# chenbinghui1/DSL

Hardware: AMD Instinct MI355X
Metric: imgs/sec training step, FCOS R50-FPN 1333x800 (higher is better)
Workload: dtype bf16; 1 GPU; FCOS R50-caffe-FPN supervised training step (BASELINE.json configs[1]), 2 x (3,800,1344) per GPU, synthetic COCO-shaped boxes, random-init weights; global_batch=2, parallelism=dp1, optimizer=SGD momentum 0.9 wd 1e-4

## Files before the change

### dsl_amd/build.py

```python
import os
import subprocess
import sys
from concurrent.futures import ThreadPoolExecutor

HERE = os.path.dirname(os.path.abspath(__file__))
CSRC = os.path.join(HERE, 'csrc')
LIBDIR = os.path.join(HERE, 'lib')
LIB = os.path.join(LIBDIR, 'libdsl_hip.so')
SOURCES = ['api.hip', 'conv.hip', 'wgrad.hip', 'misc.hip', 'fcos_loss.hip', 'optim.hip', 'detect.hip', 'rla.hip', 'datapath.hip', 'comm.hip', 'stem.hip', 'bneck.hip']
FLAGS = ['--offload-arch=gfx950', '-O3', '-std=c++17', '-fPIC', '-Wno-unused-result', '-Wno-unused-value']


def _hipcc():
    for c in (os.environ.get('HIPCC'), '/opt/rocm/bin/hipcc', 'hipcc'):
        if c and (os.path.isabs(c) and os.path.exists(c) or not os.path.isabs(c)):
            return c
    raise RuntimeError('hipcc not found')


def _stale(out, deps):
    if not os.path.exists(out):
        return True
    t = os.path.getmtime(out)
    return any(os.path.getmtime(d) > t for d in deps)


def build_lib(force=False, verbose=True):
    os.makedirs(LIBDIR, exist_ok=True)
    hdrs = [os.path.join(CSRC, 'common.hpp'), os.path.join(HERE, '..', 'include', 'dsl_hip.h')]
    srcs = [os.path.join(CSRC, s) for s in SOURCES if os.path.exists(os.path.join(CSRC, s))]
    objs = [os.path.join(LIBDIR, os.path.basename(s)[:-4] + '.o') for s in srcs]
    hipcc = _hipcc()

    def compile_one(so):
        s, o = so
        if force or _stale(o, [s] + hdrs):
            cmd = [hipcc] + FLAGS + ['-c', s, '-o', o]
            if verbose:
                print(' '.join(cmd), flush=True)
            subprocess.check_call(cmd)
        return o

    with ThreadPoolExecutor(max_workers=6) as ex:
        list(ex.map(compile_one, zip(srcs, objs)))
    if force or _stale(LIB, objs):
        cmd = [hipcc, '--offload-arch=gfx950', '-shared', '-fPIC', '-Wl,--no-undefined'] + objs + ['-ldl', '-o', LIB]
        if verbose:
            print(' '.join(cmd), flush=True)
        subprocess.check_call(cmd)
    return LIB


if __name__ == '__main__':
    build_lib(force='--force' in sys.argv)
    print(LIB)
```

### dsl_amd/csrc/conv.hip

```cpp
#include <stdlib.h>
#include <algorithm>

#include <mutex>
#include <type_traits>
#include <vector>

#include "common.hpp"

namespace {

constexpr int BPX = 128;
constexpr int BK = 64;

struct ConvK {
  int nseg, n;
  int gh[DSL_MAX_SEG], gw[DSL_MAX_SEG], sh[DSL_MAX_SEG], sw[DSL_MAX_SEG];
  int dh[DSL_MAX_SEG], dw[DSL_MAX_SEG], ah[DSL_MAX_SEG], aw[DSL_MAX_SEG];
  int pxstart[DSL_MAX_SEG + 1];
  long long soff[DSL_MAX_SEG], doff[DSL_MAX_SEG], aoff[DSL_MAX_SEG];
  int cs, cd, ldd, lda, ldm, kh, kw, stride, pad, mode, os, flags;
  int lds;
  int ktiles, kc;
  int ident;
  int addfast;
  int dbg;
  int splits, kt_per_split, cd_pad;
  int gx, gy, xcd_chunk;
  float* ws;
  long long wrow;
  const uint16_t* src;
  const uint16_t* wgt;
  void* dst;
  const float* scale;
  const float* bias;
  const uint16_t* addend;
  const uint16_t* mask;
  float* gnws;
  const uint16_t* gnx;
  const float* gngamma;
  const float* gnbeta;
  const float* gnstats;
};

__device__ __forceinline__ u32x4 relu_bf16x8(u32x4 v) {
#pragma unroll
  for (int i = 0; i < 4; ++i) {
    uint32_t w = v[i];
    uint32_t neg = (w >> 15) & 0x00010001u;
    v[i] = w & ~(neg * 0xffffu);
  }
  return v;
}

struct PixRow {
  long long base;
  int y, x, sh, sw;
  bool ok;
};

__device__ __forceinline__ void lds_barrier() {
  asm volatile("s_waitcnt lgkmcnt(0)\n\ts_barrier" ::: "memory");
}

__device__ __forceinline__ void decode_pixel(const ConvK& p, int gp, int& seg, int& img, int& y, int& x) {
  seg = 0;
#pragma unroll
  for (int s = 1; s < DSL_MAX_SEG; ++s)
    if (s < p.nseg && gp >= p.pxstart[s]) seg = s;
  const int q = gp - p.pxstart[seg];
  const int hw = p.gh[seg] * p.gw[seg];
  img = q / hw;
  const int rem = q - img * hw;
  y = rem / p.gw[seg];
  x = rem - y * p.gw[seg];
}


__device__ __forceinline__ void conv_epilogue4(const ConvK& p, long long dpix, long long apix, int co, float v[4]) {
  const bool out_f32 = (p.flags & DSL_CONV_OUT_F32) != 0;
  const bool relu_out = (p.flags & DSL_CONV_RELU_OUT) != 0;
  const bool mask_first = (p.flags & DSL_CONV_MASK_FIRST) != 0 && p.mask != nullptr;
  const bool mask_last = (p.flags & DSL_CONV_MASK_LAST) != 0 && p.mask != nullptr;
  const bool has_mask = mask_first || mask_last;
  if (co + 3 < p.cd) {
    if (p.scale) {
      const f32x4 s4 = *reinterpret_cast<const f32x4*>(p.scale + co);
#pragma unroll
      for (int e = 0; e < 4; ++e) v[e] *= s4[e];
    }
    if (p.bias) {
      const f32x4 b4 = *reinterpret_cast<const f32x4*>(p.bias + co);
#pragma unroll
      for (int e = 0; e < 4; ++e) v[e] += b4[e];
    }
    float m[4] = {1.f, 1.f, 1.f, 1.f};
    if (has_mask) {
      const u32x2 mm = *reinterpret_cast<const u32x2*>(p.mask + dpix * p.ldm + co);
      m[0] = bflo(mm[0]) > 0.f ? 1.f : 0.f;
      m[1] = bfhi(mm[0]) > 0.f ? 1.f : 0.f;
// ... 199 lines not shown
    for (int i = 0; i < 8; ++i) v[i] = fmaxf(v[i], 0.f);
  }
  const u32x4 o = {pack2bf(v[0], v[1]), pack2bf(v[2], v[3]), pack2bf(v[4], v[5]), pack2bf(v[6], v[7])};
  *reinterpret_cast<u32x4*>(e.dst + (long long)gp * e.ldd) = o;
}

__device__ __forceinline__ void conv_out_index(const ConvK& p, int gp, long long& dpix, long long& apix) {
  if (p.ident) {
    dpix = gp;
    apix = gp;
    return;
  }
  int seg, img, y, x;
  decode_pixel(p, gp, seg, img, y, x);
  const int oy = y * p.os, ox = x * p.os;
  dpix = p.doff[seg] + ((long long)img * p.dh[seg] + oy) * p.dw[seg] + ox;
  apix = dpix;
  if (p.flags & DSL_CONV_ADD_UPSAMPLE) {
    const int ay = (oy * p.ah[seg]) / p.dh[seg], ax = (ox * p.aw[seg]) / p.dw[seg];
    apix = p.aoff[seg] + ((long long)img * p.ah[seg] + ay) * p.aw[seg] + ax;
  }
}

__global__ __launch_bounds__(256) void conv_splitk_epilogue_kernel(const ConvK p) {
  const int totpx = p.pxstart[p.nseg];
  const int c4 = p.cd_pad / 4;
  const long long total = (long long)totpx * c4;
  for (long long i = (long long)blockIdx.x * blockDim.x + threadIdx.x; i < total; i += (long long)gridDim.x * blockDim.x) {
    const int gp = (int)(i / c4);
    const int co = (int)(i - (long long)gp * c4) * 4;
    if (co >= p.cd) continue;
    f32x4 s = {0.f, 0.f, 0.f, 0.f};
    for (int sp = 0; sp < p.splits; ++sp)
      s += *reinterpret_cast<const f32x4*>(p.ws + ((long long)sp * totpx + gp) * p.cd_pad + co);
    long long dpix, apix;
    conv_out_index(p, gp, dpix, apix);
    float v[4] = {s[0], s[1], s[2], s[3]};
    conv_epilogue4(p, dpix, apix, co, v);
  }
}

template <int BCO, bool SMALLC>
__global__ __launch_bounds__(256) void conv_gemm_kernel(const ConvK p) {
  extern __shared__ __attribute__((aligned(16))) unsigned char smem[];
  constexpr int TILE_W = BCO * BK * 2;
  constexpr int TILE_X = BPX * BK * 2;
  constexpr int STAGE = TILE_W + TILE_X;
  constexpr int WM = BCO / 2;
  constexpr int CT = WM / 32;
  constexpr int WPASS = BCO / 32;

  const int tid = threadIdx.x, lane = tid & 63, wave = tid >> 6;
  const int wave_co = wave >> 1, wave_px = wave & 1;
  const int co0 = blockIdx.x * BCO;
  const int px0 = blockIdx.y * BPX;
  const int totpx = p.pxstart[p.nseg];
  const int lrow = tid >> 3, chunk = tid & 7;
// ... 729 lines not shown
      continue;
    }
#pragma nounroll
    for (int id = tid; id < CPX * GPR; id += T) {
      const int pl = id / GPR, cg = id - pl * GPR;
      const int gp = px0 + (pl >> 5) * (32 * PT) + pt * 32 + (pl & 31);
      const int co = co0 + cg * 8;
      if (gp >= totpx || co >= p.cd) continue;
      const f32x4 lo = *reinterpret_cast<const f32x4*>(smem + pl * ROWB + cg * 32);
      const f32x4 hi = *reinterpret_cast<const f32x4*>(smem + pl * ROWB + cg * 32 + 16);
      float v[8] = {lo[0], lo[1], lo[2], lo[3], hi[0], hi[1], hi[2], hi[3]};
#ifdef DSL_ABLATE_BUILD
      if ((p.dbg & 512) && v[0] != 12345.678f) continue;
#endif
      long long dpix, apix;
      conv_out_index(p, gp, dpix, apix);
      conv_epilogue8a(p, dpix, apix, co, v, aff);
    }
    stamp(3 + 3 * pt);
  }
}

template <int BCO, int BPX, int WCO, int WPX, int NST, bool SMC = false, bool GNB = false>
__global__ __launch_bounds__(64 * WCO * WPX) void conv_pipe_kernel(const ConvK p) {
  extern __shared__ __attribute__((aligned(16))) unsigned char smem[];
  constexpr int T = 64 * WCO * WPX;
  constexpr int RPP = T / 8;
  constexpr int WPASS = BCO / RPP, XPASS = BPX / RPP;
  constexpr int TILE_W = BCO * 128;
  constexpr int STAGE = (BCO + BPX) * 128;
  constexpr int PT = BPX / WPX / 32;
  constexpr int CT = BCO / WCO / 32;
  constexpr int HB = 1;
  static_assert(BCO == WCO * CT * 32 && CT >= 1, "cout tiles per wave");
  static_assert(BCO % RPP == 0 && BPX % RPP == 0 && (BPX / WPX) % 32 == 0, "tile/thread mismatch");

  const int tid = threadIdx.x, lane = tid & 63;
  const int wave = __builtin_amdgcn_readfirstlane(tid >> 6);
  const int wave_co = wave / WPX, wave_px = wave % WPX;
#ifdef DSL_ABLATE_BUILD
  if (p.dbg & 128) return;
#endif
  const int wi = (int)(blockIdx.x & 7) * p.xcd_chunk + (int)(blockIdx.x >> 3);
  if ((int)(blockIdx.x >> 3) >= p.xcd_chunk || wi >= p.gx * p.gy * p.splits) return;
  const int bz = wi / (p.gx * p.gy);
  const int rem_t = wi - bz * (p.gx * p.gy);
  const int by = rem_t / p.gx;
  const int co0 = (rem_t - by * p.gx) * BCO;
  const int px0 = by * BPX;
  const int totpx = p.pxstart[p.nseg];
  const int dt = tid, dwave = wave;
  const int lrow = dt >> 3;
  const int chunk = (dt & 7) ^ ((dt >> 4) & 7);

  const unsigned margin = (unsigned)(p.kw * p.lds * 2);
  const __amdgpu_buffer_rsrc_t rs_src =
      __builtin_amdgcn_make_buffer_rsrc((void*)(reinterpret_cast<const unsigned char*>(p.src) - margin), 0, 0x7fffffff, 0x00020000);
  const __amdgpu_buffer_rsrc_t rs_wgt = __builtin_amdgcn_make_buffer_rsrc((void*)p.wgt, 0, 0x7fffffff, 0x00020000);

  const int kt0 = bz * p.kt_per_split;
#ifdef DSL_ABLATE_BUILD
  const int kt1 = (p.dbg & 8) ? kt0 + 1 : min(kt0 + p.kt_per_split, p.ktiles);
#else
  const int kt1 = min(kt0 + p.kt_per_split, p.ktiles);
#endif
  int cidx = kt0 % p.kc;
  int tap_r = (kt0 / p.kc) / p.kw, tap_s = (kt0 / p.kc) % p.kw;

  unsigned r_cur[XPASS], r_step[XPASS], r_mask[XPASS];
  int r_y[XPASS], r_x[XPASS], r_hw[XPASS];
#pragma unroll
  for (int i = 0; i < XPASS; ++i) {
    const int gp = px0 + lrow + RPP * i;
    int seg = 0, img = 0, y = 0, x = 0;
    const bool ok = gp < totpx;
    if (ok) decode_pixel(p, gp, seg, img, y, x);
    const int sh = p.sh[seg], sw = p.sw[seg];
    if (SMC) {
      r_y[i] = ok ? y * p.stride - p.pad : -100000;
      r_x[i] = x * p.stride - p.pad;
      r_hw[i] = (sh << 16) | sw;
      r_cur[i] = (unsigned)(((int)(p.soff[seg]) + img * sh * sw + r_y[i] * sw + r_x[i]) * 16) + margin;
      r_step[i] = r_mask[i] = 0;
      continue;
    }
    const int row0 = p.mode == 0 ? y * p.stride - p.pad : y + p.pad;
    const int col0 = p.mode == 0 ? x * p.stride - p.pad : x + p.pad - (p.kw - 1);
    unsigned m = 0;
    for (int r = 0; r < p.kh; ++r) {
      const int sy = p.mode == 0 ? row0 + r : row0 - r;
      if (ok && (unsigned)sy < (unsigned)sh) m |= 1u << r;
    }
    for (int s_ = 0; s_ < p.kw; ++s_) {
      const int sx = p.mode == 0 ? col0 + s_ : x + p.pad - s_;
      if (ok && (unsigned)sx < (unsigned)sw) m |= 0x100u << s_;
    }
    r_mask[i] = m;
    const unsigned pitch = (unsigned)(sw * p.lds * 2);
    r_step[i] = p.mode == 0 ? pitch : 0u - pitch;
    const unsigned base = (unsigned)(((int)(p.soff[seg]) + img * sh * sw + row0 * sw + col0) * p.lds + chunk * 8) * 2u + margin;
    r_cur[i] = base + (unsigned)tap_r * r_step[i];
  }
  const unsigned w_voff = (unsigned)(lrow * (int)p.wrow + chunk * 8) * 2u;
  const unsigned w_pass = (unsigned)(RPP * (int)p.wrow) * 2u;
  unsigned w_soff = (unsigned)(co0 * (int)p.wrow + kt0 * BK) * 2u;

  constexpr int LPT = WPASS + XPASS;
  constexpr int P0 = (LPT + 1) / 3;
  constexpr int P1 = P0 + (LPT - P0 + 1) / 2;
  int kt_next = kt0;
  unsigned t_sel = (1u << tap_r) | (0x100u << tap_s);
  unsigned t_soff = (unsigned)((p.mode == 0 ? tap_s : p.kw - 1 - tap_s) * p.lds * 2 + cidx * 128);
  unsigned t_wv = w_voff;
  int c_left = p.kc - cidx;
  unsigned r_v[XPASS];
#pragma unroll
  for (int i = 0; i < XPASS; ++i) r_v[i] = (r_mask[i] & t_sel) == t_sel ? r_cur[i] : 0x80000000u;
  auto pieces = [&](auto lo_c, auto hi_c, const unsigned ld_off) {
    constexpr int LO = decltype(lo_c)::value, HI = decltype(hi_c)::value;
    unsigned char* stage = smem + ld_off;
    const bool live = kt_next < kt1;
    const unsigned s_off = t_soff;
    const unsigned wv = t_wv;
    int s_tr = 0, s_ts = 0;
    bool s_ok = false;
    if (SMC) {
      const int tap = kt_next * 8 + chunk;
      s_tr = tap / p.kw;
      s_ts = tap - s_tr * p.kw;
      s_ok = live && tap < p.kh * p.kw;
    }
#pragma unroll
    for (int j = LO; j < HI; ++j) {
#ifdef DSL_ABLATE_BUILD
      if (p.dbg & (j < XPASS ? 1 : 2)) continue;
#endif
      if (j < XPASS) {
        unsigned v, so;
        if (SMC) {
          const int sh = r_hw[j] >> 16, sw = r_hw[j] & 0xffff;
          const bool in = s_ok && (unsigned)(r_y[j] + s_tr) < (unsigned)sh && (unsigned)(r_x[j] + s_ts) < (unsigned)sw;
          v = in ? r_cur[j] + (unsigned)((s_tr * sw + s_ts) * 16) : 0x80000000u;
          so = 0;
        } else {
          v = r_v[j];
          so = s_off;
        }
        __builtin_amdgcn_raw_ptr_buffer_load_lds(rs_src, (lptr_t)(stage + TILE_W + (j * RPP + dwave * 8) * 128), 16, v, so, 0, 0);
      } else {
        const int i = j - XPASS;
        __builtin_amdgcn_raw_ptr_buffer_load_lds(rs_wgt, (lptr_t)(stage + (i * RPP + dwave * 8) * 128), 16, wv,
                                                 w_soff + i * w_pass, 0, 0);
      }
    }
    if (HI == LPT) {
      ++kt_next;
      w_soff += BK * 2;
      if (--c_left != 0) {
        t_soff += 128;
      } else {
        c_left = p.kc;
        const bool s_wrap = tap_s + 1 == p.kw;
        tap_s = s_wrap ? 0 : tap_s + 1;
        if (s_wrap) {
          ++tap_r;
#pragma unroll
          for (int i = 0; i < XPASS; ++i) r_cur[i] += r_step[i];
        }
        t_sel = (1u << tap_r) | (0x100u << tap_s);
        t_soff = (unsigned)((p.mode == 0 ? tap_s : p.kw - 1 - tap_s) * p.lds * 2);
#pragma unroll
        for (int i = 0; i < XPASS; ++i) r_v[i] = (r_mask[i] & t_sel) == t_sel ? r_cur[i] : 0x80000000u;
      }
      if (__builtin_expect(kt_next >= kt1, 0)) {
        asm volatile("" ::: "memory");
        t_sel = 0xffffffffu;
        t_wv = 0x80000000u;
#pragma unroll
        for (int i = 0; i < XPASS; ++i) r_v[i] = 0x80000000u;
      }
    }
  };
  using c0_t = std::integral_constant<int, 0>;
  using cp0_t = std::integral_constant<int, P0>;
  using cp1_t = std::integral_constant<int, P1>;
  using clpt_t = std::integral_constant<int, LPT>;

#ifdef DSL_ABLATE_BUILD
  if (p.dbg & 256) return;
#endif
  f32x16 acc[CT][PT];
#pragma unroll
  for (int a = 0; a < CT; ++a)
#pragma unroll
    for (int b = 0; b < PT; ++b)
#pragma unroll
      for (int j = 0; j < 16; ++j) acc[a][b][j] = 0.f;

  const int frow = lane & 31, fhalf = lane >> 5;
  const int fswz = (frow >> 1) & 7;
  const int a_off = (wave_co * (32 * CT) + frow) * 128;
  const int b_off = TILE_W + (wave_px * (32 * PT) + frow) * 128;
  bf16x8 fa[2][CT], fb[2][PT];
  auto lds_read = [&](const unsigned char* base, int kk, int f) {
#ifdef DSL_ABLATE_BUILD
    if (p.dbg & 64) return;
#endif
    const int coff = ((2 * kk + fhalf) ^ fswz) << 4;
#pragma unroll
    for (int ct = 0; ct < CT; ++ct) fa[f][ct] = *reinterpret_cast<const bf16x8*>(base + a_off + ct * 32 * 128 + coff);
#pragma unroll
    for (int pt = 0; pt < PT; ++pt) fb[f][pt] = *reinterpret_cast<const bf16x8*>(base + b_off + pt * 32 * 128 + coff);
// ... 11 lines not shown
    for (int ct = 0; ct < CT; ++ct)
      if (ct < n) mma_half(f, ct);
  };
  auto mma = [&](int f) { mma_upto(f, CT); };

  static_assert((NST - 1) * LPT <= 63, "vmcnt range");
#ifdef DSL_TRACE_BUILD
  const bool tr_on = wi == p.dbg;
  int tr_it = 0;
  unsigned long long* tr_lds = reinterpret_cast<unsigned long long*>(smem + NST * STAGE) + wave * (kTraceIters * 8);
#define TR(i)                                                                                  \
  do {                                                                                         \
    __builtin_amdgcn_sched_barrier(0);                                                         \
    if (tr_on && tr_it < kTraceIters) {                                                        \
      const unsigned long long t_ = __builtin_amdgcn_s_memtime();                              \
      if (lane == 0) tr_lds[tr_it * 8 + (i)] = t_;                                             \
    }                                                                                          \
    __builtin_amdgcn_sched_barrier(0);                                                         \
  } while (0)
#else
#define TR(i) do {} while (0)
#endif
  if (WCO * WPX == 8 && wave >= 4) __builtin_amdgcn_s_setprio(1);
#pragma unroll
  for (int s = 0; s < NST - 1; ++s) pieces(c0_t{}, clpt_t{}, (unsigned)(s * STAGE));
  pieces(c0_t{}, cp0_t{}, (unsigned)((NST - 1) * STAGE));
  wait_vmcnt<(NST - 2) * LPT + P0>();
  __builtin_amdgcn_s_barrier();
  lds_read(smem, 0, 0);
  unsigned slot = 0;
  unsigned pslot = (NST - 1) * STAGE;
  for (int kt = kt0; kt < kt1 - 1; ++kt) {
    const unsigned char* base = smem + slot;
    const unsigned nslot = (slot + STAGE == NST * STAGE) ? 0u : slot + STAGE;
    TR(0);
#ifdef DSL_ABLATE_BUILD
    if (p.dbg & 1024) {
      unsigned d_ = (unsigned)kt;
#pragma unroll
      for (int q = 0; q < 32; ++q) asm volatile("s_add_u32 %0, %0, 1" : "+s"(d_));
      if (d_ == 0x7fffffffu) return;
    }
    if (p.dbg & 2048) {
      unsigned d_ = (unsigned)lane;
#pragma unroll
      for (int q = 0; q < 32; ++q) asm volatile("v_add_u32 %0, %0, 1" : "+v"(d_));
      if (d_ == 0x7fffffffu) return;
    }
// ... 59 lines not shown
      const unsigned long long t_ = __builtin_amdgcn_s_memtime();                              \
      if (lane == 0) tre_lds[(i)] = t_;                                                        \
    }                                                                                          \
    __builtin_amdgcn_sched_barrier(0);                                                         \
  } while (0)
  TRE(0);
  auto trace_dump = [&]() {
    asm volatile("s_waitcnt vmcnt(0)" ::: "memory");
    TRE(15);
    if (tr_on) {
      __syncthreads();
      for (int i = tid; i < 8 * kTraceIters * 8 + 8 * 16; i += T)
        g_conv_trace[i] = reinterpret_cast<const unsigned long long*>(smem + NST * STAGE)[i];
      if (tid == 0) g_conv_trace[8 * kTraceIters * 8 + 8 * 16] = (unsigned long long)(WCO * WPX);
    }
  };
#else
#define TRE(i) do {} while (0)
#endif
#ifdef DSL_ABLATE_BUILD
  if (p.dbg & 16) return;
#endif

  if (p.splits > 1) {
#pragma unroll
    for (int pt = 0; pt < PT; ++pt) {
      const int gp = px0 + wave_px * (32 * PT) + pt * 32 + (lane & 31);
      if (gp >= totpx) continue;
      float* row = p.ws + ((long long)bz * totpx + gp) * p.cd_pad;
#pragma unroll
      for (int ct = 0; ct < CT; ++ct)
#pragma unroll
        for (int g = 0; g < 4; ++g) {
          const int co = co0 + wave_co * (32 * CT) + ct * 32 + 8 * g + 4 * (lane >> 5);
          f32x4 o = {acc[ct][pt][4 * g], acc[ct][pt][4 * g + 1], acc[ct][pt][4 * g + 2], acc[ct][pt][4 * g + 3]};
          *reinterpret_cast<f32x4*>(row + co) = o;
        }
    }
    return;
  }

#ifdef DSL_TRACE_BUILD
  conv_tile_epilogue<BCO, BPX, WCO, WPX, CT, PT, NST * STAGE, GNB>(p, acc, smem, co0, px0, totpx, [&](int i_) { TRE(i_); });
#else
  conv_tile_epilogue<BCO, BPX, WCO, WPX, CT, PT, NST * STAGE, GNB>(p, acc, smem, co0, px0, totpx, [](int) {});
#endif
#ifdef DSL_TRACE_BUILD
  trace_dump();
#endif
#undef TRE
}

typedef int v8i32 __attribute__((ext_vector_type(8)));
template <int BCO, int BPX, int WCO, int WPX, int NST>
__global__ __launch_bounds__(64 * WCO * WPX) void conv_f8_kernel(const ConvK p) {
  constexpr bool SMC = false;
  extern __shared__ __attribute__((aligned(16))) unsigned char smem[];
  constexpr int T = 64 * WCO * WPX;
  constexpr int RPP = T / 8;
  constexpr int WPASS = BCO / RPP, XPASS = BPX / RPP;
  constexpr int TILE_W = BCO * 128;
  constexpr int STAGE = (BCO + BPX) * 128;
  constexpr int PT = BPX / WPX / 32;
  static_assert(BCO / WCO == 64, "each wave owns 64 couts");
  static_assert(BCO % RPP == 0 && BPX % RPP == 0 && (BPX / WPX) % 32 == 0, "tile/thread mismatch");

  const int tid = threadIdx.x, lane = tid & 63;
  const int wave = __builtin_amdgcn_readfirstlane(tid >> 6);
  const int wave_co = wave / WPX, wave_px = wave % WPX;
  const int wi = (int)(blockIdx.x & 7) * p.xcd_chunk + (int)(blockIdx.x >> 3);
  if ((int)(blockIdx.x >> 3) >= p.xcd_chunk || wi >= p.gx * p.gy * p.splits) return;
  const int bz = wi / (p.gx * p.gy);
  const int rem_t = wi - bz * (p.gx * p.gy);
  const int by = rem_t / p.gx;
  const int co0 = (rem_t - by * p.gx) * BCO;
  const int px0 = by * BPX;
  const int totpx = p.pxstart[p.nseg];
  const int lrow = tid >> 3;
  const int chunk = (tid & 7) ^ ((tid >> 4) & 7);

  const unsigned margin = (unsigned)(p.kw * p.lds);
  const __amdgpu_buffer_rsrc_t rs_src =
      __builtin_amdgcn_make_buffer_rsrc((void*)(reinterpret_cast<const unsigned char*>(p.src) - margin), 0, 0x7fffffff, 0x00020000);
  const __amdgpu_buffer_rsrc_t rs_wgt = __builtin_amdgcn_make_buffer_rsrc((void*)p.wgt, 0, 0x7fffffff, 0x00020000);

  const int kt0 = bz * p.kt_per_split;
  const int kt1 = min(kt0 + p.kt_per_split, p.ktiles);
  int cidx = kt0 % p.kc;
  int tap_r = (kt0 / p.kc) / p.kw, tap_s = (kt0 / p.kc) % p.kw;

  unsigned r_cur[XPASS], r_step[XPASS], r_mask[XPASS];
  int r_y[XPASS], r_x[XPASS], r_hw[XPASS];
#pragma unroll
  for (int i = 0; i < XPASS; ++i) {
    const int gp = px0 + lrow + RPP * i;
    int seg = 0, img = 0, y = 0, x = 0;
    const bool ok = gp < totpx;
    if (ok) decode_pixel(p, gp, seg, img, y, x);
    const int sh = p.sh[seg], sw = p.sw[seg];
    if (SMC) {
      r_y[i] = ok ? y * p.stride - p.pad : -100000;
      r_x[i] = x * p.stride - p.pad;
      r_hw[i] = (sh << 16) | sw;
      r_cur[i] = (unsigned)(((int)(p.soff[seg]) + img * sh * sw + r_y[i] * sw + r_x[i]) * 16) + margin;
      r_step[i] = r_mask[i] = 0;
      continue;
    }
    const int row0 = p.mode == 0 ? y * p.stride - p.pad : y + p.pad;
    const int col0 = p.mode == 0 ? x * p.stride - p.pad : x + p.pad - (p.kw - 1);
    unsigned m = 0;
    for (int r = 0; r < p.kh; ++r) {
      const int sy = p.mode == 0 ? row0 + r : row0 - r;
      if (ok && (unsigned)sy < (unsigned)sh) m |= 1u << r;
    }
    for (int s_ = 0; s_ < p.kw; ++s_) {
      const int sx = p.mode == 0 ? col0 + s_ : x + p.pad - s_;
      if (ok && (unsigned)sx < (unsigned)sw) m |= 0x100u << s_;
    }
    r_mask[i] = m;
    const unsigned pitch = (unsigned)(sw * p.lds);
    r_step[i] = p.mode == 0 ? pitch : 0u - pitch;
    const unsigned base = (unsigned)(((int)(p.soff[seg]) + img * sh * sw + row0 * sw + col0) * p.lds + chunk * 16) + margin;
    r_cur[i] = base + (unsigned)tap_r * r_step[i];
  }
  const unsigned w_voff = (unsigned)(lrow * (int)p.wrow + chunk * 16);
  const unsigned w_pass = (unsigned)(RPP * (int)p.wrow);
  unsigned w_soff = (unsigned)(co0 * (int)p.wrow + kt0 * 128);

  constexpr int LPT = WPASS + XPASS;
  constexpr int P0 = (LPT + 1) / 3;
  constexpr int P1 = P0 + (LPT - P0 + 1) / 2;
  int kt_next = kt0;
  int ld_slot = 0;
  auto pieces = [&](auto lo_c, auto hi_c) {
    constexpr int LO = decltype(lo_c)::value, HI = decltype(hi_c)::value;
    unsigned char* stage = smem + ld_slot * STAGE;
    const bool live = kt_next < kt1;
    const unsigned sel = live ? ((1u << tap_r) | (0x100u << tap_s)) : 0xffffffffu;
    const unsigned s_off = (unsigned)((p.mode == 0 ? tap_s : p.kw - 1 - tap_s) * p.lds + cidx * 128);
    const unsigned wv = live ? w_voff : 0x80000000u;
    int s_tr = 0, s_ts = 0;
    bool s_ok = false;
    if (SMC) {
      const int tap = kt_next * 8 + chunk;
      s_tr = tap / p.kw;
      s_ts = tap - s_tr * p.kw;
      s_ok = live && tap < p.kh * p.kw;
    }
#pragma unroll
    for (int j = LO; j < HI; ++j) {
      if (j < XPASS) {
        unsigned v, so;
        if (SMC) {
          const int sh = r_hw[j] >> 16, sw = r_hw[j] & 0xffff;
          const bool in = s_ok && (unsigned)(r_y[j] + s_tr) < (unsigned)sh && (unsigned)(r_x[j] + s_ts) < (unsigned)sw;
          v = in ? r_cur[j] + (unsigned)((s_tr * sw + s_ts) * 16) : 0x80000000u;
          so = 0;
        } else {
          v = (r_mask[j] & sel) == sel ? r_cur[j] : 0x80000000u;
          so = s_off;
        }
        __builtin_amdgcn_raw_ptr_buffer_load_lds(rs_src, (lptr_t)(stage + TILE_W + (j * RPP + wave * 8) * 128), 16, v, so, 0, 0);
      } else {
        const int i = j - XPASS;
        __builtin_amdgcn_raw_ptr_buffer_load_lds(rs_wgt, (lptr_t)(stage + (i * RPP + wave * 8) * 128), 16, wv,
                                                 w_soff + i * w_pass, 0, 0);
      }
    }
    if (HI == LPT) {
      ++kt_next;
      ld_slot = (ld_slot + 1 == NST) ? 0 : ld_slot + 1;
      w_soff += BK * 2;
      const bool c_wrap = cidx + 1 == p.kc;
      const bool s_wrap = c_wrap && tap_s + 1 == p.kw;
      cidx = c_wrap ? 0 : cidx + 1;
      tap_s = s_wrap ? 0 : (c_wrap ? tap_s + 1 : tap_s);
      tap_r += s_wrap ? 1 : 0;
      const unsigned adv = s_wrap ? 0xffffffffu : 0u;
#pragma unroll
      for (int i = 0; i < XPASS; ++i) r_cur[i] += r_step[i] & adv;
    }
  };
  using c0_t = std::integral_constant<int, 0>;
  using cp0_t = std::integral_constant<int, P0>;
  using cp1_t = std::integral_constant<int, P1>;
  using clpt_t = std::integral_constant<int, LPT>;

  f32x16 acc[2][PT];
#pragma unroll
  for (int a = 0; a < 2; ++a)
#pragma unroll
    for (int b = 0; b < PT; ++b)
#pragma unroll
      for (int j = 0; j < 16; ++j) acc[a][b][j] = 0.f;

  const int frow = lane & 31, fhalf = lane >> 5;
  const int fswz = (frow >> 1) & 7;
// ... 39 lines not shown
    mma_half(1, 0);
    sched_stage<2 * PT, 2 * (2 + PT), LPT - P0>();
    sched_stage<PT, 0, 0>();
    __builtin_amdgcn_sched_barrier(0);
    asm volatile("s_waitcnt lgkmcnt(0)" ::: "memory");
    wait_vmcnt<(NST - 2) * LPT>();
    __builtin_amdgcn_s_barrier();
    lds_read(smem + nslot * STAGE, 0, 0);
    pieces(c0_t{}, cp0_t{});
    mma_half(1, 1);
    __builtin_amdgcn_sched_group_barrier(0x100, 2 * (2 + PT), 0);
    sched_stage<PT, 0, P0>();
    slot = nslot;
  }
  {
    const unsigned char* base = smem + slot * STAGE;
    lds_read(base, 1, 1);
    mma(0);
    mma(1);
    sched_stage<2 * PT, 2 * (2 + PT), 0>();
  }
  wait_vmcnt<0>();

  if (p.splits > 1) {
#pragma unroll
    for (int pt = 0; pt < PT; ++pt) {
      const int gp = px0 + wave_px * (32 * PT) + pt * 32 + (lane & 31);
      if (gp >= totpx) continue;
      float* row = p.ws + ((long long)bz * totpx + gp) * p.cd_pad;
#pragma unroll
      for (int ct = 0; ct < 2; ++ct)
#pragma unroll
        for (int g = 0; g < 4; ++g) {
          const int co = co0 + wave_co * 64 + ct * 32 + 8 * g + 4 * (lane >> 5);
          f32x4 o = {acc[ct][pt][4 * g], acc[ct][pt][4 * g + 1], acc[ct][pt][4 * g + 2], acc[ct][pt][4 * g + 3]};
          *reinterpret_cast<f32x4*>(row + co) = o;
        }
    }
    return;
  }

  conv_tile_epilogue<BCO, BPX, WCO, WPX, 2, PT, NST * STAGE>(p, acc, smem, co0, px0, totpx, [](int) {});
}

}

namespace {
// ... 234 lines not shown
#ifdef DSL_TRACE_BUILD
    lds += 8 * 40 * 8 * 8 + 8 * 16 * 8;
#endif
    int prof = -1;
    if (dsl_prof_active()) prof = dsl_prof_begin(pick == 3 ? 0 : (pick == 0 ? 1 : 2), conv_algo_flops(d, px), st, conv_algo_bytes(d, px));
#define LAUNCH2(A, B, C_, D, S_)                                                                               \
  do {                                                                                                        \
    static bool attr_set = false;                                                                             \
    if (!attr_set) {                                                                                          \
      hipFuncSetAttribute((const void*)conv_glds_kernel<A, B, C_, D, S_>, hipFuncAttributeMaxDynamicSharedMemorySize, \
                          (int)lds);                                                                          \
      attr_set = true;                                                                                        \
    }                                                                                                         \
    hipLaunchKernelGGL((conv_glds_kernel<A, B, C_, D, S_>), grid, dim3(64 * C_ * D), lds, st, k);              \
  } while (0)
#define LAUNCH3(A, B, C_, D, S_)                                                                               \
  do {                                                                                                        \
    static bool attr_set3 = false;                                                                            \
    if (!attr_set3) {                                                                                         \
      hipFuncSetAttribute((const void*)conv_pipe_kernel<A, B, C_, D, S_>, hipFuncAttributeMaxDynamicSharedMemorySize, \
                          (int)lds);                                                                          \
      attr_set3 = true;                                                                                       \
    }                                                                                                         \
    hipLaunchKernelGGL((conv_pipe_kernel<A, B, C_, D, S_>), dim3(8 * k.xcd_chunk), dim3(64 * C_ * D), lds, st, k); \
  } while (0)
#define LAUNCH3G(A, B, C_, D, S_)                                                                              \
  do {                                                                                                        \
    static bool attr_set3g = false;                                                                           \
    if (!attr_set3g) {                                                                                        \
      hipFuncSetAttribute((const void*)conv_pipe_kernel<A, B, C_, D, S_, false, true>, hipFuncAttributeMaxDynamicSharedMemorySize, \
                          (int)lds);                                                                          \
      attr_set3g = true;                                                                                      \
    }                                                                                                         \
    hipLaunchKernelGGL((conv_pipe_kernel<A, B, C_, D, S_, false, true>), dim3(8 * k.xcd_chunk), dim3(64 * C_ * D), lds, st, k); \
  } while (0)
    if (fp8) {
      DSL_CHECK(!force_v2_kernel && (pick == 0 || pick == 1 || pick == 3), "dsl_conv2d: no fp8 kernel for this shape (tile config %d)", pick);
#define LAUNCH8(A, B, C_, D, S_)                                                                               \
  do {                                                                                                        \
    static bool attr_8 = false;                                                                               \
    if (!attr_8) {                                                                                            \
      hipFuncSetAttribute((const void*)conv_f8_kernel<A, B, C_, D, S_>, hipFuncAttributeMaxDynamicSharedMemorySize, \
                          (int)lds);                                                                          \
      attr_8 = true;                                                                                          \
    }                                                                                                         \
    hipLaunchKernelGGL((conv_f8_kernel<A, B, C_, D, S_>), dim3(8 * k.xcd_chunk), dim3(64 * C_ * D), lds, st, k); \
  } while (0)
      switch (pick) {
        case 0: LAUNCH8(256, 192, 4, 2, 2); break;
        case 1: LAUNCH8(256, 128, 4, 2, 3); break;
        default: LAUNCH8(128, 128, 2, 4, 2); break;
      }
#undef LAUNCH8
    } else if (force_v2_kernel) {
      switch (pick) {
        case 0: LAUNCH2(256, 192, 4, 2, 2); break;
        case 1: LAUNCH2(256, 128, 4, 2, 3); break;
        case 2: LAUNCH2(128, 256, 2, 4, 3); break;
        case 3: LAUNCH2(128, 128, 2, 2, 2); break;
        default: LAUNCH2(64, 256, 1, 4, 2); break;
      }
    } else {
      if (k.gnx) {
        if (pick == 0) LAUNCH3G(256, 192, 4, 2, 2); else LAUNCH3G(256, 128, 4, 2, 3);
      } else
      switch (pick) {
        case 0: LAUNCH3(256, 192, 4, 2, 2); break;
        case 1: LAUNCH3(256, 128, 4, 2, 3); break;
        case 2: LAUNCH3(128, 256, 2, 4, 3); break;
        case 3: LAUNCH3(128, 128, 2, 4, 2); break;
        case 4:
          if (smallc) {
            static bool a4 = false;
            if (!a4) { hipFuncSetAttribute((const void*)conv_pipe_kernel<64, 256, 1, 8, 2, true>, hipFuncAttributeMaxDynamicSharedMemorySize, (int)lds); a4 = true; }
            hipLaunchKernelGGL((conv_pipe_kernel<64, 256, 1, 8, 2, true>), dim3(8 * k.xcd_chunk), dim3(512), lds, st, k);
          } else {
            LAUNCH3(64, 256, 1, 8, 2);
          }
          break;
        case 5: LAUNCH3(128, 64, 2, 2, 3); break;
        case 6: LAUNCH3(64, 64, 1, 2, 3); break;
        default: LAUNCH3(64, 128, 1, 4, 3); break;
      }
    }
#undef LAUNCH2
#undef LAUNCH3
#undef LAUNCH3G
    dsl_prof_end(prof, st);
    if (splits > 1) {
      const long long total = (long long)px * (d->cd_pad / 4);
      int blocks = (int)((total + 255) / 256);
      if (blocks > 4096) blocks = 4096;
      hipLaunchKernelGGL(conv_splitk_epilogue_kernel, dim3(blocks), dim3(256), 0, st, k);
    }
    DSL_LAUNCH_CHECK("conv_glds_kernel");
    return 0;
  }
  const int bco = (d->cd_pad % 128 == 0) ? 128 : 64;
  dim3 grid(d->cd_pad / bco, (px + BPX - 1) / BPX);
  const size_t lds = 2 * (size_t)(bco + BPX) * BK * 2;
#define LAUNCH(BCO_, SC_)                                                                         \
  do {                                                                                            \
    static bool attr_set = false;                                                                 \
    if (!attr_set) {                                                                              \
      hipFuncSetAttribute((const void*)conv_gemm_kernel<BCO_, SC_>,                               \
                          hipFuncAttributeMaxDynamicSharedMemorySize, (int)lds);                  \
      attr_set = true;                                                                            \
    }                                                                                             \
    hipLaunchKernelGGL((conv_gemm_kernel<BCO_, SC_>), grid, dim3(256), lds, st, k);               \
  } while (0)
  int prof = -1;
  if (dsl_prof_active()) prof = dsl_prof_begin(2, conv_algo_flops(d, px), st, conv_algo_bytes(d, px));
  if (bco == 128) {
    if (smallc) LAUNCH(128, true); else LAUNCH(128, false);
  } else {
    if (smallc) LAUNCH(64, true); else LAUNCH(64, false);
// ... 14 lines not shown
```

Before: 451.3 imgs/s.

## Preload hot conv kernel args into SGPRs and issue first weight tile early

Passes the frequently used ConvK fields (pointers, grid and tiling ints) as separate leading kernel arguments and enables kernarg preloading for conv.hip, so these values arrive in SGPRs without scalar loads from the kernarg segment. The first weight tile's buffer-to-LDS loads are issued right after block-index decode, before the per-pixel decode, so weight fetch latency overlaps the prologue address setup. Pixel decode is rewritten as a branchless select over segments. This relies on a compiler flag whose effect depends on the toolchain, and it duplicates arguments in the launch.

```diff
diff --git a/dsl_amd/build.py b/dsl_amd/build.py
--- a/dsl_amd/build.py
+++ b/dsl_amd/build.py
@@ -9,6 +9,7 @@
 LIB = os.path.join(LIBDIR, 'libdsl_hip.so')
 SOURCES = ['api.hip', 'conv.hip', 'wgrad.hip', 'misc.hip', 'fcos_loss.hip', 'optim.hip', 'detect.hip', 'rla.hip', 'datapath.hip', 'comm.hip', 'stem.hip', 'bneck.hip']
 FLAGS = ['--offload-arch=gfx950', '-O3', '-std=c++17', '-fPIC', '-Wno-unused-result', '-Wno-unused-value']
+EXTRA_FLAGS = {'conv.hip': ['-mllvm', '-amdgpu-kernarg-preload-count=16']}
 
 
 def _hipcc():
@@ -35,7 +36,7 @@
     def compile_one(so):
         s, o = so
         if force or _stale(o, [s] + hdrs):
-            cmd = [hipcc] + FLAGS + ['-c', s, '-o', o]
+            cmd = [hipcc] + FLAGS + EXTRA_FLAGS.get(os.path.basename(s), []) + ['-c', s, '-o', o]
             if verbose:
                 print(' '.join(cmd), flush=True)
             subprocess.check_call(cmd)
diff --git a/dsl_amd/csrc/conv.hip b/dsl_amd/csrc/conv.hip
--- a/dsl_amd/csrc/conv.hip
+++ b/dsl_amd/csrc/conv.hip
@@ -42,6 +42,12 @@
   const float* gnstats;
 };
 
+#define CONV_HOT_PARAMS                                                                                                   \
+  const uint16_t* h_wgt, const uint16_t* h_src, const int h_wrow, const int h_xcd_chunk, const int h_gx, const int h_gy, \
+      const int h_splits, const int h_kt_per_split, const int h_ktiles, const int h_kc, const int h_kw, const int h_lds
+#define CONV_HOT_ARGS(k) \
+  (k).wgt, (k).src, (int)(k).wrow, (k).xcd_chunk, (k).gx, (k).gy, (k).splits, (k).kt_per_split, (k).ktiles, (k).kc, (k).kw, (k).lds
+
 __device__ __forceinline__ u32x4 relu_bf16x8(u32x4 v) {
 #pragma unroll
   for (int i = 0; i < 4; ++i) {
@@ -75,6 +81,28 @@
   x = rem - y * p.gw[seg];
 }
 
+__device__ __forceinline__ void decode_pixel_src(const ConvK& p, int gp, int& img, int& y, int& x, int& sh, int& sw, int& soff) {
+  int ps = p.pxstart[0], gh = p.gh[0], gw = p.gw[0];
+  sh = p.sh[0];
+  sw = p.sw[0];
+  soff = (int)p.soff[0];
+#pragma unroll
+  for (int s = 1; s < DSL_MAX_SEG; ++s) {
+    const bool in = s < p.nseg && gp >= p.pxstart[s];
+    ps = in ? p.pxstart[s] : ps;
+    gh = in ? p.gh[s] : gh;
+    gw = in ? p.gw[s] : gw;
+    sh = in ? p.sh[s] : sh;
+    sw = in ? p.sw[s] : sw;
+    soff = in ? (int)p.soff[s] : soff;
+  }
+  const int q = gp - ps;
+  const int hw = gh * gw;
+  img = q / hw;
+  const int rem = q - img * hw;
+  y = rem / gw;
+  x = rem - y * gw;
+}
 
 __device__ __forceinline__ void conv_epilogue4(const ConvK& p, long long dpix, long long apix, int co, float v[4]) {
   const bool out_f32 = (p.flags & DSL_CONV_OUT_F32) != 0;
@@ -320,17 +348,18 @@
   }
 }
 
-__global__ __launch_bounds__(256) void conv_splitk_epilogue_kernel(const ConvK p) {
-  const int totpx = p.pxstart[p.nseg];
-  const int c4 = p.cd_pad / 4;
+__global__ __launch_bounds__(256) void conv_splitk_epilogue_kernel(const float* h_ws, const int h_totpx, const int h_cd_pad, const int h_cd,
+                                                                   const int h_splits, const ConvK p) {
+  const int totpx = h_totpx;
+  const int c4 = h_cd_pad / 4;
   const long long total = (long long)totpx * c4;
   for (long long i = (long long)blockIdx.x * blockDim.x + threadIdx.x; i < total; i += (long long)gridDim.x * blockDim.x) {
     const int gp = (int)(i / c4);
     const int co = (int)(i - (long long)gp * c4) * 4;
-    if (co >= p.cd) continue;
+    if (co >= h_cd) continue;
     f32x4 s = {0.f, 0.f, 0.f, 0.f};
-    for (int sp = 0; sp < p.splits; ++sp)
-      s += *reinterpret_cast<const f32x4*>(p.ws + ((long long)sp * totpx + gp) * p.cd_pad + co);
+    for (int sp = 0; sp < h_splits; ++sp)
+      s += *reinterpret_cast<const f32x4*>(h_ws + ((long long)sp * totpx + gp) * h_cd_pad + co);
     long long dpix, apix;
     conv_out_index(p, gp, dpix, apix);
     float v[4] = {s[0], s[1], s[2], s[3]};
@@ -1106,7 +1135,7 @@
 }
 
 template <int BCO, int BPX, int WCO, int WPX, int NST, bool SMC = false, bool GNB = false>
-__global__ __launch_bounds__(64 * WCO * WPX) void conv_pipe_kernel(const ConvK p) {
+__global__ __launch_bounds__(64 * WCO * WPX) void conv_pipe_kernel(CONV_HOT_PARAMS, const ConvK p) {
   extern __shared__ __attribute__((aligned(16))) unsigned char smem[];
   constexpr int T = 64 * WCO * WPX;
   constexpr int RPP = T / 8;
@@ -1125,83 +1154,92 @@
 #ifdef DSL_ABLATE_BUILD
   if (p.dbg & 128) return;
 #endif
-  const int wi = (int)(blockIdx.x & 7) * p.xcd_chunk + (int)(blockIdx.x >> 3);
-  if ((int)(blockIdx.x >> 3) >= p.xcd_chunk || wi >= p.gx * p.gy * p.splits) return;
-  const int bz = wi / (p.gx * p.gy);
-  const int rem_t = wi - bz * (p.gx * p.gy);
-  const int by = rem_t / p.gx;
-  const int co0 = (rem_t - by * p.gx) * BCO;
+  const int wi = (int)(blockIdx.x & 7) * h_xcd_chunk + (int)(blockIdx.x >> 3);
+  if ((int)(blockIdx.x >> 3) >= h_xcd_chunk || wi >= h_gx * h_gy * h_splits) return;
+  const int bz = wi / (h_gx * h_gy);
+  const int rem_t = wi - bz * (h_gx * h_gy);
+  const int by = rem_t / h_gx;
+  const int co0 = (rem_t - by * h_gx) * BCO;
   const int px0 = by * BPX;
-  const int totpx = p.pxstart[p.nseg];
   const int dt = tid, dwave = wave;
   const int lrow = dt >> 3;
   const int chunk = (dt & 7) ^ ((dt >> 4) & 7);
 
-  const unsigned margin = (unsigned)(p.kw * p.lds * 2);
+  const unsigned margin = (unsigned)(h_kw * h_lds * 2);
   const __amdgpu_buffer_rsrc_t rs_src =
-      __builtin_amdgcn_make_buffer_rsrc((void*)(reinterpret_cast<const unsigned char*>(p.src) - margin), 0, 0x7fffffff, 0x00020000);
-  const __amdgpu_buffer_rsrc_t rs_wgt = __builtin_amdgcn_make_buffer_rsrc((void*)p.wgt, 0, 0x7fffffff, 0x00020000);
-
-  const int kt0 = bz * p.kt_per_split;
+      __builtin_amdgcn_make_buffer_rsrc((void*)(reinterpret_cast<const unsigned char*>(h_src) - margin), 0, 0x7fffffff, 0x00020000);
+  const __amdgpu_buffer_rsrc_t rs_wgt = __builtin_amdgcn_make_buffer_rsrc((void*)h_wgt, 0, 0x7fffffff, 0x00020000);
+
+  const int kt0 = bz * h_kt_per_split;
 #ifdef DSL_ABLATE_BUILD
-  const int kt1 = (p.dbg & 8) ? kt0 + 1 : min(kt0 + p.kt_per_split, p.ktiles);
+  const int kt1 = (p.dbg & 8) ? kt0 + 1 : min(kt0 + h_kt_per_split, h_ktiles);
 #else
-  const int kt1 = min(kt0 + p.kt_per_split, p.ktiles);
+  const int kt1 = min(kt0 + h_kt_per_split, h_ktiles);
 #endif
-  int cidx = kt0 % p.kc;
-  int tap_r = (kt0 / p.kc) / p.kw, tap_s = (kt0 / p.kc) % p.kw;
+  const unsigned w_voff = (unsigned)(lrow * h_wrow + chunk * 8) * 2u;
+  const unsigned w_pass = (unsigned)(RPP * h_wrow) * 2u;
+  unsigned w_soff = (unsigned)(co0 * h_wrow + kt0 * BK) * 2u;
+#pragma unroll
+  for (int i = 0; i < WPASS; ++i) {
+#ifdef DSL_ABLATE_BUILD
+    if (p.dbg & 2) continue;
+#endif
+    __builtin_amdgcn_raw_ptr_buffer_load_lds(rs_wgt, (lptr_t)(smem + (i * RPP + dwave * 8) * 128), 16, w_voff, w_soff + i * w_pass, 0, 0);
+  }
+  __builtin_amdgcn_sched_barrier(0);
+
+  const int totpx = p.pxstart[p.nseg];
+  int cidx = kt0 % h_kc;
+  int tap_r = (kt0 / h_kc) / h_kw, tap_s = (kt0 / h_kc) % h_kw;
 
   unsigned r_cur[XPASS], r_step[XPASS], r_mask[XPASS];
   int r_y[XPASS], r_x[XPASS], r_hw[XPASS];
 #pragma unroll
   for (int i = 0; i < XPASS; ++i) {
     const int gp = px0 + lrow + RPP * i;
-    int seg = 0, img = 0, y = 0, x = 0;
+    int img, y, x, sh, sw, soff;
     const bool ok = gp < totpx;
-    if (ok) decode_pixel(p, gp, seg, img, y, x);
-    const int sh = p.sh[seg], sw = p.sw[seg];
+    decode_pixel_src(p, ok ? gp : 0, img, y, x, sh, sw, soff);
     if (SMC) {
       r_y[i] = ok ? y * p.stride - p.pad : -100000;
       r_x[i] = x * p.stride - p.pad;
       r_hw[i] = (sh << 16) | sw;
-      r_cur[i] = (unsigned)(((int)(p.soff[seg]) + img * sh * sw + r_y[i] * sw + r_x[i]) * 16) + margin;
+      r_cur[i] = (unsigned)((soff + img * sh * sw + r_y[i] * sw + r_x[i]) * 16) + margin;
       r_step[i] = r_mask[i] = 0;
       continue;
     }
     const int row0 = p.mode == 0 ? y * p.stride - p.pad : y + p.pad;
-    const int col0 = p.mode == 0 ? x * p.stride - p.pad : x + p.pad - (p.kw - 1);
+    const int col0 = p.mode == 0 ? x * p.stride - p.pad : x + p.pad - (h_kw - 1);
     unsigned m = 0;
     for (int r = 0; r < p.kh; ++r) {
       const int sy = p.mode == 0 ? row0 + r : row0 - r;
       if (ok && (unsigned)sy < (unsigned)sh) m |= 1u << r;
     }
-    for (int s_ = 0; s_ < p.kw; ++s_) {
+    for (int s_ = 0; s_ < h_kw; ++s_) {
       const int sx = p.mode == 0 ? col0 + s_ : x + p.pad - s_;
       if (ok && (unsigned)sx < (unsigned)sw) m |= 0x100u << s_;
     }
     r_mask[i] = m;
-    const unsigned pitch = (unsigned)(sw * p.lds * 2);
+    const unsigned pitch = (unsigned)(sw * h_lds * 2);
     r_step[i] = p.mode == 0 ? pitch : 0u - pitch;
-    const unsigned base = (unsigned)(((int)(p.soff[seg]) + img * sh * sw + row0 * sw + col0) * p.lds + chunk * 8) * 2u + margin;
+    const unsigned base = (unsigned)((soff + img * sh * sw + row0 * sw + col0) * h_lds + chunk * 8) * 2u + margin;
     r_cur[i] = base + (unsigned)tap_r * r_step[i];
   }
-  const unsigned w_voff = (unsigned)(lrow * (int)p.wrow + chunk * 8) * 2u;
-  const unsigned w_pass = (unsigned)(RPP * (int)p.wrow) * 2u;
-  unsigned w_soff = (unsigned)(co0 * (int)p.wrow + kt0 * BK) * 2u;
 
   constexpr int LPT = WPASS + XPASS;
   constexpr int P0 = (LPT + 1) / 3;
   constexpr int P1 = P0 + (LPT - P0 + 1) / 2;
   int kt_next = kt0;
   unsigned t_sel = (1u << tap_r) | (0x100u << tap_s);
-  unsigned t_soff = (unsigned)((p.mode == 0 ? tap_s : p.kw - 1 - tap_s) * p.lds * 2 + cidx * 128);
+  unsigned t_soff = (unsigned)((p.mode == 0 ? tap_s : h_kw - 1 - tap_s) * h_lds * 2 + cidx * 128);
   unsigned t_wv = w_voff;
-  int c_left = p.kc - cidx;
+  int c_left = h_kc - cidx;
   unsigned r_v[XPASS];
 #pragma unroll
   for (int i = 0; i < XPASS; ++i) r_v[i] = (r_mask[i] & t_sel) == t_sel ? r_cur[i] : 0x80000000u;
-  auto pieces = [&](auto lo_c, auto hi_c, const unsigned ld_off) {
+  auto pieces_of = [&](auto lo_c, auto hi_c, const unsigned ld_off, auto skipw_c) {
     constexpr int LO = decltype(lo_c)::value, HI = decltype(hi_c)::value;
+    constexpr bool SKIPW = decltype(skipw_c)::value;
     unsigned char* stage = smem + ld_off;
     const bool live = kt_next < kt1;
     const unsigned s_off = t_soff;
@@ -1210,9 +1248,9 @@
     bool s_ok = false;
     if (SMC) {
       const int tap = kt_next * 8 + chunk;
-      s_tr = tap / p.kw;
-      s_ts = tap - s_tr * p.kw;
-      s_ok = live && tap < p.kh * p.kw;
+      s_tr = tap / h_kw;
+      s_ts = tap - s_tr * h_kw;
+      s_ok = live && tap < p.kh * h_kw;
     }
 #pragma unroll
     for (int j = LO; j < HI; ++j) {
@@ -1231,7 +1269,7 @@
           so = s_off;
         }
         __builtin_amdgcn_raw_ptr_buffer_load_lds(rs_src, (lptr_t)(stage + TILE_W + (j * RPP + dwave * 8) * 128), 16, v, so, 0, 0);
-      } else {
+      } else if (!SKIPW) {
         const int i = j - XPASS;
         __builtin_amdgcn_raw_ptr_buffer_load_lds(rs_wgt, (lptr_t)(stage + (i * RPP + dwave * 8) * 128), 16, wv,
                                                  w_soff + i * w_pass, 0, 0);
@@ -1243,8 +1281,8 @@
       if (--c_left != 0) {
         t_soff += 128;
       } else {
-        c_left = p.kc;
-        const bool s_wrap = tap_s + 1 == p.kw;
+        c_left = h_kc;
+        const bool s_wrap = tap_s + 1 == h_kw;
         tap_s = s_wrap ? 0 : tap_s + 1;
         if (s_wrap) {
           ++tap_r;
@@ -1252,7 +1290,7 @@
           for (int i = 0; i < XPASS; ++i) r_cur[i] += r_step[i];
         }
         t_sel = (1u << tap_r) | (0x100u << tap_s);
-        t_soff = (unsigned)((p.mode == 0 ? tap_s : p.kw - 1 - tap_s) * p.lds * 2);
+        t_soff = (unsigned)((p.mode == 0 ? tap_s : h_kw - 1 - tap_s) * h_lds * 2);
 #pragma unroll
         for (int i = 0; i < XPASS; ++i) r_v[i] = (r_mask[i] & t_sel) == t_sel ? r_cur[i] : 0x80000000u;
       }
@@ -1265,13 +1303,17 @@
       }
     }
   };
+  auto pieces = [&](auto lo_c, auto hi_c, const unsigned ld_off) { pieces_of(lo_c, hi_c, ld_off, std::false_type{}); };
   using c0_t = std::integral_constant<int, 0>;
   using cp0_t = std::integral_constant<int, P0>;
   using cp1_t = std::integral_constant<int, P1>;
   using clpt_t = std::integral_constant<int, LPT>;
 
 #ifdef DSL_ABLATE_BUILD
-  if (p.dbg & 256) return;
+  if (p.dbg & 256) {
+    wait_vmcnt<0>();
+    return;
+  }
 #endif
   f32x16 acc[CT][PT];
 #pragma unroll
@@ -1329,8 +1371,10 @@
 #define TR(i) do {} while (0)
 #endif
   if (WCO * WPX == 8 && wave >= 4) __builtin_amdgcn_s_setprio(1);
-#pragma unroll
-  for (int s = 0; s < NST - 1; ++s) pieces(c0_t{}, clpt_t{}, (unsigned)(s * STAGE));
+  static_assert(NST >= 2, "the prologue issues tile kt0 on its own");
+  pieces_of(c0_t{}, clpt_t{}, 0u, std::true_type{});
+#pragma unroll
+  for (int s = 1; s < NST - 1; ++s) pieces(c0_t{}, clpt_t{}, (unsigned)(s * STAGE));
   pieces(c0_t{}, cp0_t{}, (unsigned)((NST - 1) * STAGE));
   wait_vmcnt<(NST - 2) * LPT + P0>();
   __builtin_amdgcn_s_barrier();
@@ -1436,7 +1480,7 @@
   if (p.dbg & 16) return;
 #endif
 
-  if (p.splits > 1) {
+  if (h_splits > 1) {
 #pragma unroll
     for (int pt = 0; pt < PT; ++pt) {
       const int gp = px0 + wave_px * (32 * PT) + pt * 32 + (lane & 31);
@@ -1467,7 +1511,7 @@
 
 typedef int v8i32 __attribute__((ext_vector_type(8)));
 template <int BCO, int BPX, int WCO, int WPX, int NST>
-__global__ __launch_bounds__(64 * WCO * WPX) void conv_f8_kernel(const ConvK p) {
+__global__ __launch_bounds__(64 * WCO * WPX) void conv_f8_kernel(CONV_HOT_PARAMS, const ConvK p) {
   constexpr bool SMC = false;
   extern __shared__ __attribute__((aligned(16))) unsigned char smem[];
   constexpr int T = 64 * WCO * WPX;
@@ -1482,26 +1526,26 @@
   const int tid = threadIdx.x, lane = tid & 63;
   const int wave = __builtin_amdgcn_readfirstlane(tid >> 6);
   const int wave_co = wave / WPX, wave_px = wave % WPX;
-  const int wi = (int)(blockIdx.x & 7) * p.xcd_chunk + (int)(blockIdx.x >> 3);
-  if ((int)(blockIdx.x >> 3) >= p.xcd_chunk || wi >= p.gx * p.gy * p.splits) return;
-  const int bz = wi / (p.gx * p.gy);
-  const int rem_t = wi - bz * (p.gx * p.gy);
-  const int by = rem_t / p.gx;
-  const int co0 = (rem_t - by * p.gx) * BCO;
+  const int wi = (int)(blockIdx.x & 7) * h_xcd_chunk + (int)(blockIdx.x >> 3);
+  if ((int)(blockIdx.x >> 3) >= h_xcd_chunk || wi >= h_gx * h_gy * h_splits) return;
+  const int bz = wi / (h_gx * h_gy);
+  const int rem_t = wi - bz * (h_gx * h_gy);
+  const int by = rem_t / h_gx;
+  const int co0 = (rem_t - by * h_gx) * BCO;
   const int px0 = by * BPX;
   const int totpx = p.pxstart[p.nseg];
   const int lrow = tid >> 3;
   const int chunk = (tid & 7) ^ ((tid >> 4) & 7);
 
-  const unsigned margin = (unsigned)(p.kw * p.lds);
+  const unsigned margin = (unsigned)(h_kw * h_lds);
   const __amdgpu_buffer_rsrc_t rs_src =
-      __builtin_amdgcn_make_buffer_rsrc((void*)(reinterpret_cast<const unsigned char*>(p.src) - margin), 0, 0x7fffffff, 0x00020000);
-  const __amdgpu_buffer_rsrc_t rs_wgt = __builtin_amdgcn_make_buffer_rsrc((void*)p.wgt, 0, 0x7fffffff, 0x00020000);
-
-  const int kt0 = bz * p.kt_per_split;
-  const int kt1 = min(kt0 + p.kt_per_split, p.ktiles);
-  int cidx = kt0 % p.kc;
-  int tap_r = (kt0 / p.kc) / p.kw, tap_s = (kt0 / p.kc) % p.kw;
+      __builtin_amdgcn_make_buffer_rsrc((void*)(reinterpret_cast<const unsigned char*>(h_src) - margin), 0, 0x7fffffff, 0x00020000);
+  const __amdgpu_buffer_rsrc_t rs_wgt = __builtin_amdgcn_make_buffer_rsrc((void*)h_wgt, 0, 0x7fffffff, 0x00020000);
+
+  const int kt0 = bz * h_kt_per_split;
+  const int kt1 = min(kt0 + h_kt_per_split, h_ktiles);
+  int cidx = kt0 % h_kc;
+  int tap_r = (kt0 / h_kc) / h_kw, tap_s = (kt0 / h_kc) % h_kw;
 
   unsigned r_cur[XPASS], r_step[XPASS], r_mask[XPASS];
   int r_y[XPASS], r_x[XPASS], r_hw[XPASS];
@@ -1521,25 +1565,25 @@
       continue;
     }
     const int row0 = p.mode == 0 ? y * p.stride - p.pad : y + p.pad;
-    const int col0 = p.mode == 0 ? x * p.stride - p.pad : x + p.pad - (p.kw - 1);
+    const int col0 = p.mode == 0 ? x * p.stride - p.pad : x + p.pad - (h_kw - 1);
     unsigned m = 0;
     for (int r = 0; r < p.kh; ++r) {
       const int sy = p.mode == 0 ? row0 + r : row0 - r;
       if (ok && (unsigned)sy < (unsigned)sh) m |= 1u << r;
     }
-    for (int s_ = 0; s_ < p.kw; ++s_) {
+    for (int s_ = 0; s_ < h_kw; ++s_) {
       const int sx = p.mode == 0 ? col0 + s_ : x + p.pad - s_;
       if (ok && (unsigned)sx < (unsigned)sw) m |= 0x100u << s_;
     }
     r_mask[i] = m;
-    const unsigned pitch = (unsigned)(sw * p.lds);
+    const unsigned pitch = (unsigned)(sw * h_lds);
     r_step[i] = p.mode == 0 ? pitch : 0u - pitch;
-    const unsigned base = (unsigned)(((int)(p.soff[seg]) + img * sh * sw + row0 * sw + col0) * p.lds + chunk * 16) + margin;
+    const unsigned base = (unsigned)(((int)(p.soff[seg]) + img * sh * sw + row0 * sw + col0) * h_lds + chunk * 16) + margin;
     r_cur[i] = base + (unsigned)tap_r * r_step[i];
   }
-  const unsigned w_voff = (unsigned)(lrow * (int)p.wrow + chunk * 16);
-  const unsigned w_pass = (unsigned)(RPP * (int)p.wrow);
-  unsigned w_soff = (unsigned)(co0 * (int)p.wrow + kt0 * 128);
+  const unsigned w_voff = (unsigned)(lrow * h_wrow + chunk * 16);
+  const unsigned w_pass = (unsigned)(RPP * h_wrow);
+  unsigned w_soff = (unsigned)(co0 * h_wrow + kt0 * 128);
 
   constexpr int LPT = WPASS + XPASS;
   constexpr int P0 = (LPT + 1) / 3;
@@ -1551,15 +1595,15 @@
     unsigned char* stage = smem + ld_slot * STAGE;
     const bool live = kt_next < kt1;
     const unsigned sel = live ? ((1u << tap_r) | (0x100u << tap_s)) : 0xffffffffu;
-    const unsigned s_off = (unsigned)((p.mode == 0 ? tap_s : p.kw - 1 - tap_s) * p.lds + cidx * 128);
+    const unsigned s_off = (unsigned)((p.mode == 0 ? tap_s : h_kw - 1 - tap_s) * h_lds + cidx * 128);
     const unsigned wv = live ? w_voff : 0x80000000u;
     int s_tr = 0, s_ts = 0;
     bool s_ok = false;
     if (SMC) {
       const int tap = kt_next * 8 + chunk;
-      s_tr = tap / p.kw;
-      s_ts = tap - s_tr * p.kw;
-      s_ok = live && tap < p.kh * p.kw;
+      s_tr = tap / h_kw;
+      s_ts = tap - s_tr * h_kw;
+      s_ok = live && tap < p.kh * h_kw;
     }
 #pragma unroll
     for (int j = LO; j < HI; ++j) {
@@ -1585,8 +1629,8 @@
       ++kt_next;
       ld_slot = (ld_slot + 1 == NST) ? 0 : ld_slot + 1;
       w_soff += BK * 2;
-      const bool c_wrap = cidx + 1 == p.kc;
-      const bool s_wrap = c_wrap && tap_s + 1 == p.kw;
+      const bool c_wrap = cidx + 1 == h_kc;
+      const bool s_wrap = c_wrap && tap_s + 1 == h_kw;
       cidx = c_wrap ? 0 : cidx + 1;
       tap_s = s_wrap ? 0 : (c_wrap ? tap_s + 1 : tap_s);
       tap_r += s_wrap ? 1 : 0;
@@ -1672,7 +1716,7 @@
   }
   wait_vmcnt<0>();
 
-  if (p.splits > 1) {
+  if (h_splits > 1) {
 #pragma unroll
     for (int pt = 0; pt < PT; ++pt) {
       const int gp = px0 + wave_px * (32 * PT) + pt * 32 + (lane & 31);
@@ -1953,7 +1997,7 @@
                           (int)lds);                                                                          \
       attr_set3 = true;                                                                                       \
     }                                                                                                         \
-    hipLaunchKernelGGL((conv_pipe_kernel<A, B, C_, D, S_>), dim3(8 * k.xcd_chunk), dim3(64 * C_ * D), lds, st, k); \
+    hipLaunchKernelGGL((conv_pipe_kernel<A, B, C_, D, S_>), dim3(8 * k.xcd_chunk), dim3(64 * C_ * D), lds, st, CONV_HOT_ARGS(k), k); \
   } while (0)
 #define LAUNCH3G(A, B, C_, D, S_)                                                                              \
   do {                                                                                                        \
@@ -1963,7 +2007,7 @@
                           (int)lds);                                                                          \
       attr_set3g = true;                                                                                      \
     }                                                                                                         \
-    hipLaunchKernelGGL((conv_pipe_kernel<A, B, C_, D, S_, false, true>), dim3(8 * k.xcd_chunk), dim3(64 * C_ * D), lds, st, k); \
+    hipLaunchKernelGGL((conv_pipe_kernel<A, B, C_, D, S_, false, true>), dim3(8 * k.xcd_chunk), dim3(64 * C_ * D), lds, st, CONV_HOT_ARGS(k), k); \
   } while (0)
     if (fp8) {
       DSL_CHECK(!force_v2_kernel && (pick == 0 || pick == 1 || pick == 3), "dsl_conv2d: no fp8 kernel for this shape (tile config %d)", pick);
@@ -1975,7 +2019,7 @@
                           (int)lds);                                                                          \
       attr_8 = true;                                                                                          \
     }                                                                                                         \
-    hipLaunchKernelGGL((conv_f8_kernel<A, B, C_, D, S_>), dim3(8 * k.xcd_chunk), dim3(64 * C_ * D), lds, st, k); \
+    hipLaunchKernelGGL((conv_f8_kernel<A, B, C_, D, S_>), dim3(8 * k.xcd_chunk), dim3(64 * C_ * D), lds, st, CONV_HOT_ARGS(k), k); \
   } while (0)
       switch (pick) {
         case 0: LAUNCH8(256, 192, 4, 2, 2); break;
@@ -2004,7 +2048,7 @@
           if (smallc) {
             static bool a4 = false;
             if (!a4) { hipFuncSetAttribute((const void*)conv_pipe_kernel<64, 256, 1, 8, 2, true>, hipFuncAttributeMaxDynamicSharedMemorySize, (int)lds); a4 = true; }
-            hipLaunchKernelGGL((conv_pipe_kernel<64, 256, 1, 8, 2, true>), dim3(8 * k.xcd_chunk), dim3(512), lds, st, k);
+            hipLaunchKernelGGL((conv_pipe_kernel<64, 256, 1, 8, 2, true>), dim3(8 * k.xcd_chunk), dim3(512), lds, st, CONV_HOT_ARGS(k), k);
           } else {
             LAUNCH3(64, 256, 1, 8, 2);
           }
@@ -2022,7 +2066,7 @@
       const long long total = (long long)px * (d->cd_pad / 4);
       int blocks = (int)((total + 255) / 256);
       if (blocks > 4096) blocks = 4096;
-      hipLaunchKernelGGL(conv_splitk_epilogue_kernel, dim3(blocks), dim3(256), 0, st, k);
+      hipLaunchKernelGGL(conv_splitk_epilogue_kernel, dim3(blocks), dim3(256), 0, st, k.ws, k.pxstart[k.nseg], k.cd_pad, k.cd, k.splits, k);
     }
     DSL_LAUNCH_CHECK("conv_glds_kernel");
     return 0;
```

After: 456.1 imgs/s, median of 6. +1.1%, better.
